# fenghuayumo/DIVSHOT

Measured on AMD Instinct MI355X. Metric: train views/sec (fwd+bwd raster) at 1M splats 1920x1080, higher is better.
Workload: dtype f32; 1 GPU; C3: 1000000 splats, 1920x1080, SH degree 3, 8 views per iteration sharded over 1 GPU(s) (BASELINE config C4), 8 view(s) per GPU per step as 1 multi-view pass(es) of 8 view(s) (dvs_raster_forward_views / dvs_raster_backward_*); absgrad=True, mode=batch, stagger=False, groups=1, views_per_group=8, early_gather=False, a9_chunks=1, async_forward=True, hip_graph=False, fwd_variant=quadrant, grad_mode=0, tile_bounds=canonical, shN_layout=tiled[N/64][45][64]

## Files before the change

### divshot_amd/csrc/dvs_api.cpp

```cpp
#include <hip/hip_runtime.h>
#include <cstdio>
#include <cstdlib>
#include <cstdint>
#include <cstring>
#include <mutex>
#include <string>
#include <vector>
#include "../../include/dvs_raster.h"
#include "dvs_kernels.h"

static thread_local std::string g_last_error;
static void set_error(const char* what, hipError_t e, const char* file, int line) {
    char buf[512];
    snprintf(buf, sizeof buf, "%s: %s (%s:%d)", what, hipGetErrorString(e), file, line);
    g_last_error = buf;
}
void dvs_set_last_error(const char* msg) { g_last_error = msg ? msg : ""; }
#define HIPCHECK(expr)                                                   \
    do {                                                                 \
        hipError_t _e = (expr);                                          \
        if (_e != hipSuccess) { set_error(#expr, _e, __FILE__, __LINE__); return DVS_ERR_HIP; } \
    } while (0)

namespace {
// ... 15 lines not shown
};

DvsCam to_dev_cam(const dvs_camera& c) {
    DvsCam d;
    memcpy(d.view, c.view, sizeof d.view); memcpy(d.proj, c.proj, sizeof d.proj);
    d.tan_fovx = c.tan_fovx; d.tan_fovy = c.tan_fovy; d.focal_x = c.focal_x; d.focal_y = c.focal_y;
    memcpy(d.campos, c.campos, sizeof d.campos);
    d.width = c.width; d.height = c.height; memcpy(d.bg, c.bg, sizeof d.bg);
    return d;
}
int bits_for(uint32_t max_value) { int b = 0; while (max_value) { ++b; max_value >>= 1; } return b; }
}

struct dvs_ctx {
    int device = 0;
    size_t max_splats = 0;
    int max_w = 0, max_h = 0;
    int max_views = 1;
    int n_views = 1;
    Buf radii, splat2d, depth, flags, tiles_touched, rect, rect_sorted, key[2], ids[2];
    Buf inst_tile[2], inst_splat[2];
    uint32_t* live_splat = nullptr;
    uint32_t* live_pos = nullptr;
    bool live_lists = true;
    Buf tmp_keys, tmp_vals;
    bool export_tiles = false;
    int fe_rank_atomic = 0;
    Buf ranges_canon;
    Buf ranges, final_T, n_contrib;
    size_t fe_zero_bytes = 0;
    uint32_t fe_nbv = 0, fe_nsb = 0;
    Buf fe_state;
    Buf fe_hist;
    int fe_seg_n = -1, fe_seg_V = -1;
    uint32_t fe_seg_rows = 0;
    Buf g_rows;
    Buf dcolor;
    uint64_t* total_dev = nullptr;
    uint64_t* total_host = nullptr;
    uint64_t inst_cap = 0;
    uint64_t inst_grow_events = 0;
    bool async_T = false;
    uint64_t* rec_masks = nullptr; uint64_t rec_cap = 0;
    uint64_t overflow_seen = 0;
    dvs_fwd_state st{};
    bool have_fwd = false;
    bool keep_rows = false;
    bool rows_clean = false;
    bool rows_pending = false;
    int64_t proj_next = 0;
    struct Prep {
// ... 67 lines not shown
    const size_t state = 3 * DVS_MAX_VIEWS * sizeof(DvsSeg) + ((size_t)c->max_views * c->fe_nsb + (size_t)c->max_views * DVS_FE_MAXBINS + (size_t)c->max_views * c->fe_nbv) * 4;
    if ((r = c->fe_state.ensure(state)) != DVS_OK) return r;
    if ((r = c->fe_hist.ensure(dvs_fe_hist_words((uint64_t)c->max_splats * c->max_views, c->max_views, DVS_FE_MAXBINS) * 4)) != DVS_OK) return r;
    return DVS_OK;
}

int ensure_splat_arenas(dvs_ctx* c, size_t n) {
    int r;
#define ENS(buf, bytes) if ((r = c->buf.ensure(bytes)) != DVS_OK) return r;
    ENS(radii, n * 4) ENS(splat2d, n * 64) ENS(depth, n * 4)
    ENS(flags, n * 4) ENS(tiles_touched, n * 4) ENS(rect, n * 16) ENS(rect_sorted, n * 16)      ENS(key[0], n * 4) ENS(key[1], n * 4) ENS(ids[0], n * 4) ENS(ids[1], n * 4)
    ENS(g_rows, n * 48)
#undef ENS
    return DVS_OK;
}
int ensure_image_arenas(dvs_ctx* c, int w, int h, int views) {
    const size_t P = (size_t)w * h * views;
    const size_t tiles = (size_t)((w + DVS_TILE - 1) / DVS_TILE) * ((h + DVS_TILE - 1) / DVS_TILE) * views;
    int r;
    if ((r = c->ranges.ensure(c->fe_zero_bytes + tiles * 8)) != DVS_OK) return r;
    if ((r = c->ranges_canon.ensure(tiles * 8)) != DVS_OK) return r;
    if ((r = c->final_T.ensure(P * 4)) != DVS_OK) return r;
    if ((r = c->n_contrib.ensure(P * 4)) != DVS_OK) return r;
    return DVS_OK;
}
int ensure_instance_arenas(dvs_ctx* c, uint64_t T) {
    int r;
    if (c->inst_cap && T > c->inst_cap) ++c->inst_grow_events;
    for (int k = 0; k < 2; ++k) {
        if ((r = c->inst_tile[k].ensure(T * 4)) != DVS_OK) return r;
        if ((r = c->inst_splat[k].ensure(T * 4)) != DVS_OK) return r;
    }
    c->inst_cap = c->inst_tile[0].bytes / 4;
    for (int k = 0; k < 2; ++k) {
        if (c->inst_tile[k].bytes / 4 < c->inst_cap) c->inst_cap = c->inst_tile[k].bytes / 4;
        if (c->inst_splat[k].bytes / 4 < c->inst_cap) c->inst_cap = c->inst_splat[k].bytes / 4;
    }
    if (c->inst_cap >= (1ull << 32)) c->inst_cap = (1ull << 32) - 1;
    if ((r = c->fe_hist.ensure(dvs_fe_hist_words(c->inst_cap, c->max_views, 512) * 4)) != DVS_OK) return r;
    return DVS_OK;
}
}

extern "C" {

const char* dvs_last_error(void) { return g_last_error.c_str(); }
// ... 33 lines not shown
                    hipMemcpy(&bad, word, 4, hipMemcpyDeviceToHost) == hipSuccess)
                    probed[device] = bad == 0u ? 1 : 2;
                if (word) (void)hipFree(word);
            }
            c->fe_rank_atomic = (device < 64 && probed[device] == 1) ? 1 : 0;
        }
    }
    if (const char* v = getenv("DVS_ASYNC")) c->async_T = v[0] == '1';
    if (ensure_frontend_arenas(c) != DVS_OK ||
        ensure_splat_arenas(c, max_splats * (size_t)max_views) != DVS_OK || ensure_image_arenas(c, max_w, max_h, max_views) != DVS_OK ||
        ensure_instance_arenas(c, (uint64_t)max_splats * 4 * (uint64_t)max_views) != DVS_OK) {
        dvs_destroy(c);
        return nullptr;
    }
    return c;
}
dvs_ctx* dvs_create(int device, size_t max_splats, int max_w, int max_h) { return dvs_create_views(device, max_splats, max_w, max_h, 1); }

void dvs_destroy(dvs_ctx* c) {
    if (!c) return;
    (void)hipSetDevice(c->device);
    Buf* all[] = {&c->radii, &c->splat2d, &c->depth, &c->flags, &c->tiles_touched, &c->rect, &c->rect_sorted, &c->key[0], &c->key[1],
                  &c->ids[0], &c->ids[1], &c->inst_tile[0], &c->inst_tile[1], &c->inst_splat[0], &c->inst_splat[1],
                  &c->tmp_keys, &c->tmp_vals, &c->ranges, &c->final_T, &c->n_contrib, &c->g_rows, &c->dcolor, &c->fe_state, &c->fe_hist, &c->ranges_canon};
    for (Buf* b : all) b->release();
    if (c->total_dev) (void)hipFree(c->total_dev);
    if (c->total_host) (void)hipHostFree(c->total_host);
    for (hipEvent_t e : c->events) (void)hipEventDestroy(e);
    for (hipEvent_t e : c->probe_ev) (void)hipEventDestroy(e);
    delete c;
}

static int rect_format(const dvs_opts* opts, int tiles_x, int tiles_y) {
    if (opts->tile_bounds == DVS_TILES_TIGHT) return DVS_FE_RECT_TIGHT;
    return (tiles_x <= 255 && tiles_y <= 255) ? DVS_FE_RECT_U8 : DVS_FE_RECT_U16;
}

static int run_a2(dvs_ctx* c, hipStream_t st, const dvs_splats* p, const dvs_camera* cams, int V, const dvs_opts* opts, int64_t first, int64_t count, bool begin) {
    const int n = p->n, W = cams[0].width, H = cams[0].height;
    const int tiles_x = (W + DVS_TILE - 1) / DVS_TILE, tiles_y = (H + DVS_TILE - 1) / DVS_TILE, tiles = tiles_x * tiles_y;
    const int rect_fmt = rect_format(opts, tiles_x, tiles_y);
    DvsCams dcams;
    for (int v = 0; v < V; ++v) dcams.c[v] = to_dev_cam(cams[v]);
    if (begin) HIPCHECK(hipMemsetAsync(c->ranges.p, 0, c->fe_zero_bytes + (size_t)tiles * V * 8, st));
    HIPCHECK(dvs_launch_preprocess_fwd(st, n, p->pos, p->sh0, p->shN, p->opacity, p->scale, p->rot, dcams, V, opts->sh_degree,
                                       opts->antialias, tiles_x, tiles_y, c->radii.as<int>(), c->splat2d.as<float>(),
                                       c->depth.as<float>(), c->flags.as<uint32_t>(), c->tiles_touched.as<uint32_t>(), c->key[0].as<uint32_t>(),
// ... 84 lines not shown
        if (n > 0)
            HIPCHECK(dvs_launch_seg_binning(st, n, V, rect_fmt, fe_seg_vis(c), fe_seg_tile(c), c->ids[1].as<uint32_t>(), c->rect.as<uint32_t>(),
                                            c->rect_sorted.as<uint32_t>(), fe_block_sums(c), fe_super(c), fe_superexcl(c), tile_part,
                                            (unsigned long long*)c->total_dev, c->inst_cap, 1, tiles_x, c->inst_tile[0].as<uint32_t>(),
                                            c->inst_splat[0].as<uint32_t>(), key16));
        size_t e5 = tm.mark(); tm.span("duplicate", e4, e5);
        const bool fuse_a6 = !fe_no_fuse();
        const bool write_keys = !(fuse_a6 && c->async_T) || c->export_tiles;
        if (n > 0) {
            const uint64_t cap = c->async_T ? c->inst_cap : T;
            const uint32_t nbtot = (uint32_t)(cap / tile_part) + (uint32_t)V + 2u;
            HIPCHECK(dvs_launch_seg_sort(st, V, c->inst_tile[0].as<uint32_t>(), c->inst_splat[0].as<uint32_t>(), c->inst_tile[1].as<uint32_t>(),
                                         c->inst_splat[1].as<uint32_t>(), fe_seg_tile(c), 0, tiles > 1 ? bits_for((uint32_t)(tiles - 1)) : 1,
                                         c->async_T ? (T_expected ? T_expected : c->inst_cap) : T, tile_part, nbtot, c->fe_hist.as<uint32_t>(), fe_totals(c),
                                         (uint32_t)tiles, &icur, fuse_a6 ? ranges_ptr(c) : nullptr, write_keys ? 1 : 0, key16, c->fe_rank_atomic));
        }
        size_t e6 = tm.mark(); tm.span("tile_sort", e5, e6);
        if (fuse_a6) ranges_encoded = n > 0 ? 1 : 0;
        else HIPCHECK(dvs_launch_tile_ranges(st, T, c->inst_tile[icur].as<uint32_t>(), ranges_ptr(c), T_dev, T_expected));
        keys_written = write_keys;
        e7 = tm.mark(); tm.span("tile_ranges", e6, e7);
    }
    if (c->probe) { (void)probe_event(c, st); c->probe_kind.push_back(0); }
    c->live_splat = nullptr; c->live_pos = nullptr;
    uint64_t* rec_masks = nullptr; uint64_t rec_cap = 0;
    if (c->rec_masks && V == 1 && !c->async_T) {
        rec_masks = c->rec_masks; rec_cap = c->rec_cap;
        HIPCHECK(hipMemsetAsync(rec_masks, 0, (size_t)(T < rec_cap ? T : rec_cap) * 32, st));
    }
    if (c->live_lists && c->bwd_variant == DVS_BWD_TR) { c->live_splat = c->inst_splat[icur ^ 1].as<uint32_t>(); c->live_pos = c->inst_tile[icur ^ 1].as<uint32_t>(); }
    HIPCHECK(dvs_launch_render_fwd(st, W, H, tiles_x, tiles_y, V, ranges_ptr(c), c->inst_splat[icur].as<uint32_t>(),
                                   c->splat2d.as<float>(), bgs, out_rgb, c->final_T.as<float>(), c->n_contrib.as<uint32_t>(),
                                   c->live_splat, c->live_pos, rec_masks, rec_cap, ranges_encoded ? c->ranges_canon.as<uint32_t>() : nullptr));
    if (c->probe) (void)probe_event(c, st);
    size_t e8 = tm.mark(); tm.span("render_fwd", e7, e8);

    dvs_fwd_state& s = c->st;
    s.radii = c->radii.as<int32_t>(); s.splat2d = c->splat2d.as<float>(); s.depth = c->depth.as<float>();
    s.flags = c->flags.as<uint32_t>();
    s.tiles_touched = c->tiles_touched.as<uint32_t>();
    s.sorted_tile = keys_written ? c->inst_tile[icur].as<uint32_t>() : nullptr; s.sorted_splat = c->inst_splat[icur].as<uint32_t>();
    s.ranges = ranges_encoded ? c->ranges_canon.as<uint32_t>() : ranges_ptr(c); s.final_T = c->final_T.as<float>(); s.n_contrib = c->n_contrib.as<uint32_t>();
    s.num_rendered = c->async_T ? DVS_T_UNKNOWN : T; s.n = n; s.width = W; s.height = H; s.tiles_x = tiles_x; s.tiles_y = tiles_y;
    s._pad = 0;
    c->n_views = V;
    c->have_fwd = true;
    if (saved) *saved = s;
    if (num_rendered) *num_rendered = c->async_T ? DVS_T_UNKNOWN : T;
    if (c->timing) { HIPCHECK(hipStreamSynchronize(st)); timing_collect(c, false); }
    return DVS_OK;
}

static int check_fwd_args(dvs_ctx* c, const dvs_splats* p, const dvs_camera* cams, int V, const dvs_opts* opts, const float* out_rgb) {
    if (!c || !p || !cams || !opts || !out_rgb) { g_last_error = "dvs_raster_forward: null argument"; return DVS_ERR_INVALID; }
    if (V < 1 || V > c->max_views) { g_last_error = "dvs_raster_forward: n_views exceeds the max_views given to dvs_create_views"; return DVS_ERR_CAPACITY; }
    const dvs_camera* cam = &cams[0];
// ... 66 lines not shown
    if (!c || !out) { g_last_error = "dvs_get_view_state: null argument"; return DVS_ERR_INVALID; }
    if (!c->have_fwd || view < 0 || view >= c->n_views) { g_last_error = "dvs_get_view_state: no such view in the last forward"; return DVS_ERR_STATE; }
    dvs_fwd_state s = c->st;
    const size_t on = (size_t)view * s.n, op = (size_t)view * s.width * s.height, ot = (size_t)view * s.tiles_x * s.tiles_y;
    s.radii += on; s.splat2d += on * DVS_S2D_FLOATS; s.depth += on; s.flags += on; s.tiles_touched += on;
    s.ranges += 2 * ot; s.final_T += op; s.n_contrib += op;
    *out = s;
    return DVS_OK;
}

static int bwd_composite(dvs_ctx* c, hipStream_t st, const dvs_camera* cams, const dvs_opts* opts, const float* dL_drgb, StageTimer* tm) {
    const dvs_fwd_state& s = c->st;
    const int V = c->n_views;
    size_t e0 = tm ? tm->mark() : 0;
    if (!c->rows_clean) HIPCHECK(hipMemsetAsync(c->g_rows.p, 0, c->g_rows.bytes, st));
    c->rows_clean = false;
    size_t e1 = tm ? tm->mark() : 0;
    if (tm) tm->span("bwd_zero", e0, e1);
    float bgs[DVS_MAX_VIEWS * 3];
    for (int v = 0; v < V; ++v) for (int k = 0; k < 3; ++k) bgs[3 * v + k] = cams[v].bg[k];
    if (c->probe) { (void)probe_event(c, st); c->probe_kind.push_back(1); }
    if (c->bwd_variant == DVS_BWD_TR)
        HIPCHECK(dvs_launch_render_bwd_tr(st, s.width, s.height, s.tiles_x, s.tiles_y, V, s.ranges, s.sorted_splat, s.splat2d, bgs, s.final_T,
                                          s.n_contrib, dL_drgb, c->g_rows.as<float>(), opts->absgrad, opts->grad_mode, c->live_splat, c->live_pos));
    else
        HIPCHECK(dvs_launch_render_bwd_blocks(st, s.width, s.height, s.tiles_x, s.tiles_y, V, s.ranges, s.sorted_splat, s.splat2d,
                                              bgs, s.final_T, s.n_contrib, dL_drgb, c->g_rows.as<float>(), opts->absgrad, opts->grad_mode));
    if (c->probe) (void)probe_event(c, st);
    if (tm) { size_t e2 = tm->mark(); tm->span("render_bwd", e1, e2); }
    c->rows_pending = true;
    c->proj_next = 0;
    return DVS_OK;
}
static int bwd_project(dvs_ctx* c, hipStream_t st, const dvs_splats* p, const dvs_camera* cams, const dvs_opts* opts,
                       const dvs_splat_grads* out, StageTimer* tm) {
    const dvs_fwd_state& s = c->st;
    const int V = c->n_views, n = p->n;
    size_t e2 = tm ? tm->mark() : 0;
    if (opts->shn_layout == DVS_SHN_TILED) {
        DvsCams dcams;
        float campos[DVS_MAX_VIEWS * 3];
        for (int v = 0; v < V; ++v) { dcams.c[v] = to_dev_cam(cams[v]); for (int k = 0; k < 3; ++k) campos[3 * v + k] = cams[v].campos[k]; }
        const char* nf = getenv("DVS_A9_NO_FUSE_SH");
        const bool no_fuse = nf && nf[0] == '1';
        const bool fuse = !out->dcolor && out->sh0 && out->shN && !no_fuse;
        float* dcol = out->dcolor;
        if (!dcol && !fuse) { int r = c->dcolor.ensure((size_t)V * n * 3 * sizeof(float)); if (r != DVS_OK) return r; dcol = c->dcolor.as<float>(); }
// ... 340 lines not shown

int dvs_memcpy_d2h(dvs_ctx* c, void* host_dst, const void* dev_src, size_t bytes) {
    if (!c) return DVS_ERR_INVALID;
    HIPCHECK(hipSetDevice(c->device));
    HIPCHECK(hipDeviceSynchronize());
    HIPCHECK(hipMemcpy(host_dst, dev_src, bytes, hipMemcpyDeviceToHost));
    return DVS_OK;
}
int dvs_memcpy_h2d(dvs_ctx* c, void* dev_dst, const void* host_src, size_t bytes) {
    if (!c) return DVS_ERR_INVALID;
    HIPCHECK(hipSetDevice(c->device));
    HIPCHECK(hipMemcpy(dev_dst, host_src, bytes, hipMemcpyHostToDevice));
    return DVS_OK;
}
void* dvs_device_malloc(dvs_ctx* c, size_t bytes) {
    if (!c) return nullptr;
    void* p = nullptr;
    if (hipSetDevice(c->device) != hipSuccess || hipMalloc(&p, bytes ? bytes : 1) != hipSuccess) return nullptr;
    return p;
}
void dvs_device_free(dvs_ctx* c, void* p) { if (c && p) { (void)hipSetDevice(c->device); (void)hipFree(p); } }

}
```

### divshot_amd/csrc/dvs_kernels.h

```cpp
#pragma once
#include <hip/hip_runtime.h>
#include <stdint.h>
#include "dvs_device.h"

hipError_t dvs_launch_preprocess_fwd(hipStream_t st, int n, const float* pos, const float* sh0, const float* shN,
                                     const float* opacity, const float* scale, const float* rot, const DvsCams& cams, int n_views,
                                     int deg, int antialias, int tiles_x, int tiles_y, int* radii , float* splat2d,
                                     float* depth, uint32_t* flags,
                                     uint32_t* tiles_touched, uint32_t* depth_key, int shn_tiled,
                                     uint32_t* rect , int rect_fmt ,
                                     uint32_t* kred ,
                                     int first, int count );
hipError_t dvs_launch_preprocess_bwd(hipStream_t st, int n, const float* pos, const float* shN, const float* opacity,
                                     const float* scale, const float* rot, const DvsCam& cam, int deg, int antialias,
                                     const int* radii, const uint32_t* flags, float* grad_rows ,
                                     float* g_pos, float* g_sh0, float* g_shN, float* g_opacity, float* g_scale,
                                     float* g_rot, float* out_absgrad2d , float* out_mean2d ,
                                     float* out_dcolor , int accumulate, int rezero_rows, int shn_tiled, int grad_mode);
hipError_t dvs_launch_preprocess_bwd_views(hipStream_t st, int n, int n_views, const float* pos, const float* shN, const float* opacity,
                                           const float* scale, const float* rot, const DvsCams& cams, int deg, int antialias,
                                           const int* radii, const uint32_t* flags, float* grad_rows, float* g_pos, float* g_opacity,
                                           float* g_scale, float* g_rot, float* out_absgrad2d, float* out_mean2d, float* out_dcolor,
                                           int accumulate, int rezero_rows, int grad_mode, int first = 0, int count = -1 ,
                                           float* g_sh0 = nullptr, float* g_shN = nullptr );
// ... 59 lines not shown
void dvs_fe_block_counts(int n, uint32_t* nbv, uint32_t* nsb);
hipError_t dvs_launch_seg_init(hipStream_t st, int n, int V, uint32_t rows_per_view, DvsSeg* seg_all);
hipError_t dvs_launch_depth_sort(hipStream_t st, int n, int V, uint32_t* keys0, uint32_t* vals0, uint32_t* keys1, uint32_t* vals1,
                                 DvsSeg* seg_all, DvsSeg* seg_vis, const uint32_t* kred, uint32_t* hist, uint32_t* totals ,
                                 int rank_atomic = 0 );
hipError_t dvs_launch_seg_sort(hipStream_t st, int V, uint32_t* keys0, uint32_t* vals0, uint32_t* keys1, uint32_t* vals1, DvsSeg* seg, int bit_lo, int bits,
                               uint64_t grid_elems, uint32_t part, uint32_t nbtot, uint32_t* hist, uint32_t* totals, uint32_t key_add_per_view,
                               int* result_in, uint32_t* ranges_enc = nullptr ,
                               int write_last_keys = 1, int first_keys16 = 0 , int rank_atomic = 0);
hipError_t dvs_fe_probe_rank_atomic(hipStream_t st, uint32_t* bad_dev);
hipError_t dvs_launch_seg_binning(hipStream_t st, int n, int V, int rect_fmt, const DvsSeg* seg_vis, DvsSeg* seg_tile, const uint32_t* sorted_ids,
                                  const uint32_t* rect, uint32_t* rect_sorted, uint32_t* block_sums, unsigned long long* super, uint32_t* superexcl,
                                  uint32_t tile_part, unsigned long long* total_dev, unsigned long long capacity, int stage, int tiles_x,
                                  uint32_t* inst_tile, uint32_t* inst_splat, int key16 = 0 );

hipError_t dvs_launch_tile_ranges(hipStream_t st, uint64_t T, const uint32_t* sorted_tile, uint32_t* ranges ,
                                  const uint64_t* T_dev = nullptr, uint64_t T_expected = 0);
hipError_t dvs_launch_export_keys(hipStream_t st, uint64_t T, const uint32_t* sorted_tile, const uint32_t* sorted_splat,
                                  const float* depth, uint64_t* out_keys);

hipError_t dvs_launch_render_fwd(hipStream_t st, int W, int H, int tiles_x, int tiles_y, int n_views, const uint32_t* ranges ,
                                 const uint32_t* sorted_splat, const float* splat2d, const float* bgs, float* out_color, float* final_T,
                                 uint32_t* n_contrib, uint32_t* live_splat , uint32_t* live_pos ,
                                 uint64_t* take_masks ,
                                 uint64_t take_cap, uint32_t* ranges_out = nullptr );
enum { DVS_BWD_BLOCKS = 0 , DVS_BWD_REDUCE = 1 , DVS_BWD_MM = 2 ,
       DVS_BWD_TR = 3  };

hipError_t dvs_launch_render_bwd_tr(hipStream_t st, int W, int H, int tiles_x, int tiles_y, int n_views, const uint32_t* ranges,
                                    const uint32_t* sorted_splat, const float* splat2d, const float* bgs , const float* final_T,
                                    const uint32_t* n_contrib, const float* dL_dout, float* grad_rows, int absgrad, int grad_mode,
                                    const uint32_t* live_splat ,
                                    const uint32_t* live_pos);

hipError_t dvs_launch_render_bwd_blocks(hipStream_t st, int W, int H, int tiles_x, int tiles_y, int n_views, const uint32_t* ranges,
                                        const uint32_t* sorted_splat, const float* splat2d, const float* bgs , const float* final_T,
                                        const uint32_t* n_contrib, const float* dL_dout, float* grad_rows, int absgrad, int grad_mode);
```

### divshot_amd/csrc/render.hip

```cpp
#include "dvs_device.h"
#include "dvs_kernels.h"
#include "render_common.h"

struct __attribute__((aligned(16))) FwdLds {
    float4 a[RB];
    float4 b[RB];
    float4 c[RB];
    uint64_t qmask[RB / 64][4];
    uint32_t wlive[RB / 64];
};
__device__ __forceinline__ void lds_put(FwdLds& L, int t, float2 xy, float4 co, float3 col) {
    L.a[t] = make_float4(xy.x, xy.y, -0.72134752044448170f * co.x, -1.4426950408889634f * co.y);
    L.b[t] = make_float4(-0.72134752044448170f * co.z, co.w, col.x, col.y);
    L.c[t].x = col.z;
}

__device__ __forceinline__ bool stage_batch(FwdLds& L, const uint32_t* __restrict__ sorted_splat, uint32_t first, int cnt,
                                            const float4* __restrict__ splat2d, float tile_x0, float tile_y0, uint32_t& id_out) {
    const int t = threadIdx.x;
    uint32_t qm = 0;
    id_out = 0u;
    if (t < cnt) {
        const uint32_t id = sorted_splat[first + t];
        id_out = id;
// ... 29 lines not shown
        }
    }
    const uint64_t m0 = __ballot(qm & 1u), m1 = __ballot(qm & 2u), m2 = __ballot(qm & 4u), m3 = __ballot(qm & 8u);
    if ((t & 63) == 0) {
        uint64_t* dst = L.qmask[t >> 6];
        dst[0] = m0; dst[1] = m1; dst[2] = m2; dst[3] = m3;
    }
    return qm != 0u;
}

__device__ __forceinline__ uint64_t uniform_u64(uint64_t v) {
    const uint32_t lo = __builtin_amdgcn_readfirstlane((uint32_t)v), hi = __builtin_amdgcn_readfirstlane((uint32_t)(v >> 32));
    return ((uint64_t)hi << 32) | lo;
}

template <bool RECORD>
__global__ void __launch_bounds__(RB)
k_render_fwd(ViewBg bg_arg , int W, int H, int tiles_x, int tiles_per_view,
             int num_tiles , const uint2* __restrict__ ranges, uint2* __restrict__ ranges_out ,
             const uint32_t* __restrict__ sorted_splat, const float4* __restrict__ splat2d,
             float* __restrict__ out_color , float* __restrict__ final_T , uint32_t* __restrict__ n_contrib,
             uint32_t* __restrict__ live_splat ,
             uint32_t* __restrict__ live_pos ,
             uint64_t* __restrict__ take_masks , uint64_t take_cap) {
    __shared__ FwdLds L;
    (void)bg_arg;
    const int tile_g = tile_of_block(blockIdx.x, num_tiles);
    if (tile_g >= num_tiles) return;
    const int view = tile_g / tiles_per_view, tile = tile_g - view * tiles_per_view;
    const float3 bgv = dvs_load_bg(view);
    const float bg0 = bgv.x, bg1 = bgv.y, bg2 = bgv.z;
    out_color += (size_t)view * 3 * W * H; final_T += (size_t)view * W * H; n_contrib += (size_t)view * W * H;
    const int tx = tile % tiles_x, ty = tile / tiles_x;
    const int wave = threadIdx.x >> 6, lane = threadIdx.x & 63;
    const int px = tx * DVS_TILE + (wave & 1) * 8 + (lane & 7);
    const int py = ty * DVS_TILE + (wave >> 1) * 8 + (lane >> 3);
    const bool inside = px < W && py < H;
    const float pxf = (float)px, pyf = (float)py;
    uint2 range = ranges[tile_g];
    if (ranges_out) {
        range.x = range.y ? ~range.x : 0u;
        if (threadIdx.x == 0) ranges_out[tile_g] = range;
    }
    const int total = (int)(range.y - range.x);
    uint64_t notdone = __builtin_amdgcn_ballot_w64(inside);
    float T = 1.0f, C0 = 0.f, C1 = 0.f, C2 = 0.f;
// ... 51 lines not shown
                             "v_cmpx_ngt_f32_e32 vcc, %[amin], %[al]\n\t"
                             "v_cmp_gt_f32_e32 vcc, %[tstop], %[tt]\n\t"
                             "s_andn2_b64 %[nd], %[nd], vcc\n\t"
                             "s_andn2_b64 exec, exec, vcc\n\t"
                             "v_fmac_f32 %[c0], %[cr], %[at]\n\t"
                             "v_fmac_f32 %[c1], %[cg], %[at]\n\t"
                             "v_fmac_f32 %[c2], %[cbl], %[at]\n\t"
                             "v_sub_f32 %[T], %[T], %[at]\n\t"
                             "v_mov_b32 %[last], %[idx]\n\t"
                             "s_mov_b64 exec, %[ee]"
                             : [c0] "+v"(C0), [c1] "+v"(C1), [c2] "+v"(C2), [T] "+v"(T), [last] "+v"(last), [nd] "+s"(notdone)
                             : [p2] "v"(p2), [al] "v"(alpha), [tt] "v"(test_T), [cr] "v"(B.z), [cg] "v"(B.w), [cbl] "v"(cb), [at] "v"(aT), [idx] "s"(idx),
                               [amin] "s"(DVS_ALPHA_MIN), [tstop] "s"(DVS_T_STOP), [ee] "s"(exec_entry)
                             : "vcc", "scc");
                if (RECORD) {
                    const uint64_t took = nd_before & __builtin_amdgcn_ballot_w64(!(p2 > 0.f)) & __builtin_amdgcn_ballot_w64(!(alpha < DVS_ALPHA_MIN)) &
                                          ~__builtin_amdgcn_ballot_w64(test_T < DVS_T_STOP);
                    const uint64_t pos = (uint64_t)range.x + (uint64_t)(idx - 1u);
                    if (lane == 0 && pos < take_cap) take_masks[pos * 4 + wave] = took;
                }
            }
        }
    }
    if (inside) {
        const size_t P = (size_t)W * H, pix = (size_t)py * W + px;
        final_T[pix] = T;
        n_contrib[pix] = last;
        out_color[pix] = C0 + T * bg0;
        out_color[P + pix] = C1 + T * bg1;
        out_color[2 * P + pix] = C2 + T * bg2;
    }
}


hipError_t dvs_launch_render_fwd(hipStream_t st, int W, int H, int tiles_x, int tiles_y, int n_views, const uint32_t* ranges,
                                 const uint32_t* sorted_splat, const float* splat2d, const float* bgs, float* out_color, float* final_T,
                                 uint32_t* n_contrib, uint32_t* live_splat, uint32_t* live_pos, uint64_t* take_masks, uint64_t take_cap, uint32_t* ranges_out) {
    const int tiles_pv = tiles_x * tiles_y, num_tiles = tiles_pv * n_views;
    if (num_tiles <= 0) return hipSuccess;
    const int grid = ((num_tiles + 7) >> 3) << 3;
    if (take_masks)
        hipLaunchKernelGGL(k_render_fwd<true>, dim3(grid), dim3(RB), 0, st, make_view_bg(n_views, bgs), W, H, tiles_x, tiles_pv, num_tiles,
                           (const uint2*)ranges, (uint2*)ranges_out, sorted_splat, (const float4*)splat2d, out_color, final_T, n_contrib, live_splat, live_pos, take_masks, take_cap);
    else
        hipLaunchKernelGGL(k_render_fwd<false>, dim3(grid), dim3(RB), 0, st, make_view_bg(n_views, bgs), W, H, tiles_x, tiles_pv, num_tiles,
                           (const uint2*)ranges, (uint2*)ranges_out, sorted_splat, (const float4*)splat2d, out_color, final_T, n_contrib, live_splat, live_pos, (uint64_t*)nullptr, (uint64_t)0);
    return hipGetLastError();
}
```

### divshot_amd/csrc/render_tr.hip

```cpp
#include "dvs_device.h"
#include "dvs_kernels.h"
#include "render_common.h"

#define TR_SLOTS 4
#define TR_SS 136
#define TR_MINW 6

template <int BK>
struct __attribute__((aligned(16))) TrLds {
    float4 ea[BK + 1];
    float4 eb[BK + 1];
    float4 ec[BK + 1];
    uint2 idop[2][BK];
    uint8_t list[(BK + 1) * 16];
    uint32_t cnt[16];
    uint32_t blast[16];
};

template <int BK>
__device__ __forceinline__ uint32_t tr_load_id(const uint32_t* __restrict__ sorted_splat, uint32_t first, int cnt) {
    const int e = threadIdx.x % BK;
    return e < cnt ? sorted_splat[first + e] : 0u;
}
template <int BK>
// ... 40 lines not shown
        uint32_t rk, len;
        if (BK == 64) {
            rk = __builtin_amdgcn_mbcnt_hi((uint32_t)(m >> 32), __builtin_amdgcn_mbcnt_lo((uint32_t)m, 0u));
            len = (uint32_t)__popcll(m);
        } else {
            const uint32_t lo = (uint32_t)m, hi = (uint32_t)(m >> 32);
            const bool up = lane >= 32;
            rk = up ? __builtin_amdgcn_mbcnt_hi(hi, 0u) : __builtin_amdgcn_mbcnt_lo(lo, 0u);
            len = (uint32_t)__popc(up ? hi : lo);
        }
        if (hit) L.list[(rk + 1u) * 16u + (uint32_t)(b0 + i)] = (uint8_t)e;
        if (e == 0) L.cnt[b0 + i] = len;
    }
}

template <bool ABSGRAD, bool LINEAGE, int BK>
__global__ void __launch_bounds__(RB, TR_MINW)
k_render_bwd_tr(ViewBg bg_arg , int W, int H, int tiles_x, int tiles_per_view,
                int num_tiles , const uint2* __restrict__ ranges,
                const uint32_t* __restrict__ sorted_splat, const float4* __restrict__ splat2d,
                const float* __restrict__ final_T, const uint32_t* __restrict__ n_contrib, const float* __restrict__ dL_dout ,
                float* __restrict__ grow ,
                const uint32_t* __restrict__ live_splat ,
                const uint32_t* __restrict__ live_pos ) {
    __shared__ TrLds<BK> L;
    __shared__ __attribute__((aligned(16))) float s_tab[4][(BK + 1) * 12];
    __shared__ __attribute__((aligned(16))) float s_tb[4][TR_SLOTS * TR_SS];
    (void)bg_arg;
    const int tile_g = tile_of_block(blockIdx.x, num_tiles);
    if (tile_g >= num_tiles) return;
    const int view = tile_g / tiles_per_view, tile = tile_g - view * tiles_per_view;
    const float3 bgv = dvs_load_bg(view);
    final_T += (size_t)view * W * H; n_contrib += (size_t)view * W * H; dL_dout += (size_t)view * 3 * W * H;
    const int tx = tile % tiles_x, ty = tile / tiles_x;
    const int wave = threadIdx.x >> 6, lane = threadIdx.x & 63;
    const size_t P = (size_t)W * H;
    const int g1 = lane >> 4, pi = lane & 15;
    const int bx1 = 2 * (wave & 1) + (g1 & 1), by1 = 2 * (wave >> 1) + (g1 >> 1), blk1 = by1 * 4 + bx1;
    const int px = tx * DVS_TILE + 4 * bx1 + (pi & 3), py = ty * DVS_TILE + 4 * by1 + (pi >> 2);
    const bool inside = px < W && py < H;
    const size_t pix = (size_t)py * W + px;
    const float pxf = (float)px, pyf = (float)py;
    const uint2 range = ranges[tile_g];
    const int r2 = lane >> 4, s2 = (lane >> 2) & 3, g2 = lane & 3;
    const int bx2 = 2 * (wave & 1) + (g2 & 1), by2 = 2 * (wave >> 1) + (g2 >> 1);
    const int X0 = tx * DVS_TILE + 4 * bx2, Y0 = ty * DVS_TILE + 4 * by2 + r2;
    const float X0f = (float)X0, Y0f = (float)Y0;
    float d2[4][3];
    if ((W & 3) == 0) {
        const bool in2 = X0 < W && Y0 < H;
        const size_t q = (size_t)Y0 * W + X0;
#pragma unroll
        for (int c = 0; c < 3; ++c) {
            const float4 v = in2 ? *reinterpret_cast<const float4*>(dL_dout + c * P + q) : make_float4(0.f, 0.f, 0.f, 0.f);
            d2[0][c] = v.x; d2[1][c] = v.y; d2[2][c] = v.z; d2[3][c] = v.w;
        }
    } else {
#pragma unroll
        for (int x = 0; x < 4; ++x) {
            const bool in2 = X0 + x < W && Y0 < H;
            const size_t q = (size_t)Y0 * W + X0 + x;
#pragma unroll
            for (int c = 0; c < 3; ++c) d2[x][c] = in2 ? dL_dout[c * P + q] : 0.f;
        }
    }
    const int perm_r = (r2 == 1) ? 2 : (r2 == 2) ? 1 : r2;
    const int xaddr = (lane ^ 32) << 2;
    const int jaddr = (16 * g2) << 2;
    const uint32_t jshift = 8u * (uint32_t)(TR_SLOTS - 1 - s2);

    const float T_final = inside ? final_T[pix] : 0.f;
    uint32_t last = inside ? n_contrib[pix] : 0u;
    if (live_pos) {
        if (last > 0u) last = live_pos[range.x + last - 1u] + 1u;
        sorted_splat = live_splat;
    }
    float dLp0 = 0.f, dLp1 = 0.f, dLp2 = 0.f;
    if (inside) { dLp0 = dL_dout[pix]; dLp1 = dL_dout[P + pix]; dLp2 = dL_dout[2 * P + pix]; }
    const float bg_dot = (bgv.x * dLp0 + bgv.y * dLp1) + bgv.z * dLp2;

    uint32_t bmax = last;
#pragma unroll
    for (int d = 8; d >= 1; d >>= 1) bmax = max(bmax, (uint32_t)__shfl_xor((int)bmax, d, 64));
    if (pi == 0) L.blast[blk1] = bmax;
    for (int e = threadIdx.x; e < (BK + 1) * 12; e += RB) reinterpret_cast<float4*>(&s_tab[0][0])[e] = make_float4(0.f, 0.f, 0.f, 0.f);
    if (threadIdx.x < 16) L.list[threadIdx.x] = (uint8_t)BK;
    if (threadIdx.x == 0) { L.ea[BK] = make_float4(0.f, 0.f, 0.f, 0.f); L.eb[BK] = make_float4(0.f, 0.f, 0.f, 0.f); L.ec[BK] = make_float4(0.f, 0.f, 0.f, 0.f); }
    __syncthreads();
    uint32_t todo = 0;
#pragma unroll
    for (int g = 0; g < 16; ++g) todo = max(todo, L.blast[g]);
    if (todo == 0) return;

    float T = T_final;
    float D = T_final * bg_dot;
    const uint32_t tb_m0 = (uint32_t)__builtin_amdgcn_readfirstlane((int)(uint32_t)(uintptr_t)&s_tb[wave][0]);
    typedef __attribute__((address_space(3))) float lds_float;
    typedef float tr_v4f __attribute__((ext_vector_type(4)));
    typedef __attribute__((address_space(3))) const tr_v4f lds_cv4f;
    uint32_t tbr_a = (uint32_t)(uintptr_t)&s_tb[wave][TR_SS * s2 + 16 * g2 + 4 * r2];
    uint32_t tabw_a = (uint32_t)(uintptr_t)&s_tab[wave][perm_r];
    asm("" : "+v"(tbr_a), "+v"(tabw_a));
    const uint8_t* const lbase = &L.list[0];

    auto flush = [&](uint32_t jpack) {
        const uint32_t jp = (uint32_t)__builtin_amdgcn_ds_bpermute(jaddr, (int)jpack);
        const int j = (int)((jp >> jshift) & 0xffu);
        const tr_v4f V_ = *(lds_cv4f*)tbr_a, W_ = *(lds_cv4f*)(tbr_a + 256u);
        const float4 V = make_float4(V_.x, V_.y, V_.z, V_.w), Wv = make_float4(W_.x, W_.y, W_.z, W_.w);
        const float2 mean = *reinterpret_cast<const float2*>(&L.ea[j]);
        const float4 cq = L.ec[j];
        asm("" : : "v"(cq.x));
        const float Dx = mean.x - X0f, Dy = mean.y - Y0f;
        const float A0 = (V.x + V.y) + (V.z + V.w);
        const float B0 = __builtin_fmaf(3.f, V.w, __builtin_fmaf(2.f, V.z, V.y));
// ... 20 lines not shown
        const float h3 = swap32_add(v[6], v[7]);
        float h4, h5;
        if (ABSGRAD) {
            h4 = swap32_add(v[8], v[9]);
            h5 = v[10] + __int_as_float(__builtin_amdgcn_ds_bpermute(xaddr, __float_as_int(v[10])));
        } else {
            h4 = v[8] + __int_as_float(__builtin_amdgcn_ds_bpermute(xaddr, __float_as_int(v[8])));
            h5 = 0.f;
        }
        const float q0 = swap16_add(h0, h1), q1 = swap16_add(h2, h3), q2 = swap16_add(h4, h5);
        uint32_t slot_a;
        asm("v_mad_u32_u24 %0, %1, 48, %2" : "=v"(slot_a) : "v"(j), "v"(tabw_a));
        lds_float* const slot = (lds_float*)slot_a;
#pragma unroll
        for (int g = 0; g < 4; ++g) {
            if (g2 == g) { slot[0] += q0; slot[4] += q1; slot[8] += q2; }
            __builtin_amdgcn_wave_barrier();
            asm volatile("" ::: "memory");
        }
    };

    const int nbatch = (int)((todo + BK - 1) / BK);
    const float tile_x0 = (float)(tx * DVS_TILE), tile_y0 = (float)(ty * DVS_TILE);
    uint32_t id_stage = tr_load_id<BK>(sorted_splat, range.x + (nbatch - 1) * BK, min(BK, (int)todo - (nbatch - 1) * BK));
    for (int b = nbatch - 1; b >= 0; --b) {
        const int base = b * BK;
        const int cnt = min(BK, (int)todo - base);
        tr_stage<BK>(L, splat2d, id_stage, cnt, base, b & 1, tile_x0, tile_y0);
        __syncthreads();
        const int len = (int)L.cnt[blk1];
        int nmax = len;
        nmax = max(nmax, __shfl_xor(nmax, 16, 64));
        nmax = max(nmax, __shfl_xor(nmax, 32, 64));
        nmax = __builtin_amdgcn_readfirstlane(nmax);
        const int lastb = (int)min(last, (uint32_t)(base + BK)) - base;
        uint32_t p = (uint32_t)len * 16u + (uint32_t)blk1;
        uint32_t jn = lbase[p];
        asm("" : "+v"(jn));
        uint32_t jpack = 0;
        int nslot = 0;
#pragma unroll 1
        for (int it = 0; it < nmax; ++it) {
            const int j = (int)jn;
            jpack = (jpack << 8) | (uint32_t)j;
            const bool below_last = j < lastb;
            const float4 ea = L.ea[j];
            const float4 eb = L.eb[j];
// ... 27 lines not shown
                tbw[TR_SS * nslot] = 0.f; tbw[TR_SS * nslot + 64] = 0.f;
                jpack = (jpack << 8) | (uint32_t)BK;
            }
            flush(jpack);
        }
        __syncthreads();
        if (b > 0) id_stage = tr_load_id<BK>(sorted_splat, range.x + (b - 1) * BK, BK);
        for (int e = threadIdx.x; e < cnt * 12; e += RB) {
            const float val = (s_tab[0][e] + s_tab[1][e]) + (s_tab[2][e] + s_tab[3][e]);
            if (val != 0.f) {
                const int ent = e / 12, comp = e - 12 * ent;
                const uint2 io = L.idop[b & 1][ent];
                const float sc = (comp == 5 || (comp >= 6 && comp <= 8)) ? 1.f : __uint_as_float(io.y);
                if (comp < 11) atomicAdd(&grow[(size_t)io.x * 12 + comp], val * sc);
            }
            s_tab[0][e] = 0.f; s_tab[1][e] = 0.f; s_tab[2][e] = 0.f; s_tab[3][e] = 0.f;
        }
    }
}

hipError_t dvs_launch_render_bwd_tr(hipStream_t st, int W, int H, int tiles_x, int tiles_y, int n_views, const uint32_t* ranges,
                                    const uint32_t* sorted_splat, const float* splat2d, const float* bgs, const float* final_T,
                                    const uint32_t* n_contrib, const float* dL_dout, float* grad_rows, int absgrad, int grad_mode,
                                    const uint32_t* live_splat, const uint32_t* live_pos) {
    const int tiles_pv = tiles_x * tiles_y, num_tiles = tiles_pv * n_views;
    if (num_tiles <= 0) return hipSuccess;
    const int grid = ((num_tiles + 7) >> 3) << 3;
    const int lineage = grad_mode == 1 ? 1 : 0;
#define DVS_TR(A, LN, BKV)                                                                                                              \
    hipLaunchKernelGGL((k_render_bwd_tr<A, LN, BKV>), dim3(grid), dim3(RB), 0, st, make_view_bg(n_views, bgs), W, H, tiles_x, tiles_pv, \
                       num_tiles, (const uint2*)ranges, sorted_splat, (const float4*)splat2d, final_T, n_contrib, dL_dout, grad_rows, live_splat, live_pos)
#define DVS_TR_B(BKV)                                                                                   \
    do {                                                                                                \
        if (absgrad) { if (lineage) DVS_TR(true, true, BKV); else DVS_TR(true, false, BKV); }           \
        else { if (lineage) DVS_TR(false, true, BKV); else DVS_TR(false, false, BKV); }                 \
    } while (0)
    DVS_TR_B(64);
#undef DVS_TR_B
#undef DVS_TR
    return hipGetLastError();
}
```

Before: 1824 views/s.

## Hand off live-list pixel counts and per-block maxima from forward to backward

The forward render now converts each pixel's contributor count into a live-list position and writes it to a new per-pixel buffer. It also reduces per-4x4-block maxima and writes them to a per-tile array. The backward tile kernel reads these precomputed values instead of doing a dependent gather through live_pos, a shuffle reduction and an LDS pass. This lets it exit early for empty tiles and prefetch the first id batch before the barrier. The cost is extra global writes and a barrier in the forward pass, plus two new image-sized buffers.

```diff
diff --git a/divshot_amd/csrc/dvs_api.cpp b/divshot_amd/csrc/dvs_api.cpp
--- a/divshot_amd/csrc/dvs_api.cpp
+++ b/divshot_amd/csrc/dvs_api.cpp
@@ -61,11 +61,14 @@
     Buf inst_tile[2], inst_splat[2];
     uint32_t* live_splat = nullptr;
     uint32_t* live_pos = nullptr;
+    uint32_t* n_contrib_live = nullptr;
+    uint32_t* tile_blast = nullptr;
     bool live_lists = true;
     Buf tmp_keys, tmp_vals;
     bool export_tiles = false;
     int fe_rank_atomic = 0;
     Buf ranges_canon;
+    Buf handoff_px, handoff_tile;
     Buf ranges, final_T, n_contrib;
     size_t fe_zero_bytes = 0;
     uint32_t fe_nbv = 0, fe_nsb = 0;
@@ -179,6 +182,8 @@
     if ((r = c->ranges_canon.ensure(tiles * 8)) != DVS_OK) return r;
     if ((r = c->final_T.ensure(P * 4)) != DVS_OK) return r;
     if ((r = c->n_contrib.ensure(P * 4)) != DVS_OK) return r;
+    if ((r = c->handoff_px.ensure(P * 4)) != DVS_OK) return r;
+    if ((r = c->handoff_tile.ensure(tiles * 64)) != DVS_OK) return r;
     return DVS_OK;
 }
 int ensure_instance_arenas(dvs_ctx* c, uint64_t T) {
@@ -258,7 +263,8 @@
     (void)hipSetDevice(c->device);
     Buf* all[] = {&c->radii, &c->splat2d, &c->depth, &c->flags, &c->tiles_touched, &c->rect, &c->rect_sorted, &c->key[0], &c->key[1],
                   &c->ids[0], &c->ids[1], &c->inst_tile[0], &c->inst_tile[1], &c->inst_splat[0], &c->inst_splat[1],
-                  &c->tmp_keys, &c->tmp_vals, &c->ranges, &c->final_T, &c->n_contrib, &c->g_rows, &c->dcolor, &c->fe_state, &c->fe_hist, &c->ranges_canon};
+                  &c->tmp_keys, &c->tmp_vals, &c->ranges, &c->final_T, &c->n_contrib, &c->g_rows, &c->dcolor, &c->fe_state, &c->fe_hist, &c->ranges_canon,
+                  &c->handoff_px, &c->handoff_tile};
     for (Buf* b : all) b->release();
     if (c->total_dev) (void)hipFree(c->total_dev);
     if (c->total_host) (void)hipHostFree(c->total_host);
@@ -389,16 +395,19 @@
         e7 = tm.mark(); tm.span("tile_ranges", e6, e7);
     }
     if (c->probe) { (void)probe_event(c, st); c->probe_kind.push_back(0); }
-    c->live_splat = nullptr; c->live_pos = nullptr;
+    c->live_splat = nullptr; c->live_pos = nullptr; c->n_contrib_live = nullptr; c->tile_blast = nullptr;
     uint64_t* rec_masks = nullptr; uint64_t rec_cap = 0;
     if (c->rec_masks && V == 1 && !c->async_T) {
         rec_masks = c->rec_masks; rec_cap = c->rec_cap;
         HIPCHECK(hipMemsetAsync(rec_masks, 0, (size_t)(T < rec_cap ? T : rec_cap) * 32, st));
     }
-    if (c->live_lists && c->bwd_variant == DVS_BWD_TR) { c->live_splat = c->inst_splat[icur ^ 1].as<uint32_t>(); c->live_pos = c->inst_tile[icur ^ 1].as<uint32_t>(); }
+    if (c->live_lists && c->bwd_variant == DVS_BWD_TR) {
+        c->live_splat = c->inst_splat[icur ^ 1].as<uint32_t>(); c->live_pos = c->inst_tile[icur ^ 1].as<uint32_t>();
+        c->n_contrib_live = c->handoff_px.as<uint32_t>(); c->tile_blast = c->handoff_tile.as<uint32_t>();
+    }
     HIPCHECK(dvs_launch_render_fwd(st, W, H, tiles_x, tiles_y, V, ranges_ptr(c), c->inst_splat[icur].as<uint32_t>(),
                                    c->splat2d.as<float>(), bgs, out_rgb, c->final_T.as<float>(), c->n_contrib.as<uint32_t>(),
-                                   c->live_splat, c->live_pos, rec_masks, rec_cap, ranges_encoded ? c->ranges_canon.as<uint32_t>() : nullptr));
+                                   c->live_splat, c->live_pos, c->n_contrib_live, c->tile_blast, rec_masks, rec_cap, ranges_encoded ? c->ranges_canon.as<uint32_t>() : nullptr));
     if (c->probe) (void)probe_event(c, st);
     size_t e8 = tm.mark(); tm.span("render_fwd", e7, e8);
 
@@ -511,7 +520,8 @@
     if (c->probe) { (void)probe_event(c, st); c->probe_kind.push_back(1); }
     if (c->bwd_variant == DVS_BWD_TR)
         HIPCHECK(dvs_launch_render_bwd_tr(st, s.width, s.height, s.tiles_x, s.tiles_y, V, s.ranges, s.sorted_splat, s.splat2d, bgs, s.final_T,
-                                          s.n_contrib, dL_drgb, c->g_rows.as<float>(), opts->absgrad, opts->grad_mode, c->live_splat, c->live_pos));
+                                          s.n_contrib, dL_drgb, c->g_rows.as<float>(), opts->absgrad, opts->grad_mode, c->live_splat, c->live_pos,
+                                          c->n_contrib_live, c->tile_blast));
     else
         HIPCHECK(dvs_launch_render_bwd_blocks(st, s.width, s.height, s.tiles_x, s.tiles_y, V, s.ranges, s.sorted_splat, s.splat2d,
                                               bgs, s.final_T, s.n_contrib, dL_drgb, c->g_rows.as<float>(), opts->absgrad, opts->grad_mode));
@@ -898,3 +908,13 @@
 void dvs_device_free(dvs_ctx* c, void* p) { if (c && p) { (void)hipSetDevice(c->device); (void)hipFree(p); } }
 
 }
+
+namespace dvs_test {
+__attribute__((visibility("default"))) int handoff_state(dvs_ctx* c, const uint32_t** live_pos, const uint32_t** n_contrib_live, const uint32_t** tile_blast) {
+    if (!c || !c->have_fwd) return DVS_ERR_STATE;
+    if (live_pos) *live_pos = c->live_pos;
+    if (n_contrib_live) *n_contrib_live = c->n_contrib_live;
+    if (tile_blast) *tile_blast = c->tile_blast;
+    return DVS_OK;
+}
+}
diff --git a/divshot_amd/csrc/dvs_kernels.h b/divshot_amd/csrc/dvs_kernels.h
--- a/divshot_amd/csrc/dvs_kernels.h
+++ b/divshot_amd/csrc/dvs_kernels.h
@@ -105,6 +105,7 @@
 hipError_t dvs_launch_render_fwd(hipStream_t st, int W, int H, int tiles_x, int tiles_y, int n_views, const uint32_t* ranges ,
                                  const uint32_t* sorted_splat, const float* splat2d, const float* bgs, float* out_color, float* final_T,
                                  uint32_t* n_contrib, uint32_t* live_splat , uint32_t* live_pos ,
+                                 uint32_t* n_contrib_live , uint32_t* tile_blast ,
                                  uint64_t* take_masks ,
                                  uint64_t take_cap, uint32_t* ranges_out = nullptr );
 enum { DVS_BWD_BLOCKS = 0 , DVS_BWD_REDUCE = 1 , DVS_BWD_MM = 2 ,
@@ -114,7 +115,7 @@
                                     const uint32_t* sorted_splat, const float* splat2d, const float* bgs , const float* final_T,
                                     const uint32_t* n_contrib, const float* dL_dout, float* grad_rows, int absgrad, int grad_mode,
                                     const uint32_t* live_splat ,
-                                    const uint32_t* live_pos);
+                                    const uint32_t* live_pos, const uint32_t* n_contrib_live , const uint32_t* tile_blast);
 
 hipError_t dvs_launch_render_bwd_blocks(hipStream_t st, int W, int H, int tiles_x, int tiles_y, int n_views, const uint32_t* ranges,
                                         const uint32_t* sorted_splat, const float* splat2d, const float* bgs , const float* final_T,
diff --git a/divshot_amd/csrc/render.hip b/divshot_amd/csrc/render.hip
--- a/divshot_amd/csrc/render.hip
+++ b/divshot_amd/csrc/render.hip
@@ -75,6 +75,8 @@
              float* __restrict__ out_color , float* __restrict__ final_T , uint32_t* __restrict__ n_contrib,
              uint32_t* __restrict__ live_splat ,
              uint32_t* __restrict__ live_pos ,
+             uint32_t* __restrict__ n_contrib_live ,
+             uint32_t* __restrict__ tile_blast ,
              uint64_t* __restrict__ take_masks , uint64_t take_cap) {
     __shared__ FwdLds L;
     (void)bg_arg;
@@ -172,8 +174,23 @@
             }
         }
     }
+    const size_t P = (size_t)W * H, pix = (size_t)py * W + px;
+    if (n_contrib_live) {
+        __threadfence_block();
+        __syncthreads();
+        const uint32_t ll = last ? live_pos[range.x + last - 1u] + 1u : 0u;
+        if (inside) n_contrib_live[(size_t)view * P + pix] = ll;
+        uint32_t bmax = ll;
+        bmax = max(bmax, (uint32_t)__shfl_xor((int)bmax, 1, 64));
+        bmax = max(bmax, (uint32_t)__shfl_xor((int)bmax, 2, 64));
+        bmax = max(bmax, (uint32_t)__shfl_xor((int)bmax, 8, 64));
+        bmax = max(bmax, (uint32_t)__shfl_xor((int)bmax, 16, 64));
+        if ((lane & 27) == 0) {
+            const int bx = 2 * (wave & 1) + ((lane >> 2) & 1), by = 2 * (wave >> 1) + (lane >> 5);
+            tile_blast[(size_t)tile_g * 16 + (size_t)(by * 4 + bx)] = bmax;
+        }
+    }
     if (inside) {
-        const size_t P = (size_t)W * H, pix = (size_t)py * W + px;
         final_T[pix] = T;
         n_contrib[pix] = last;
         out_color[pix] = C0 + T * bg0;
@@ -185,15 +202,17 @@
 
 hipError_t dvs_launch_render_fwd(hipStream_t st, int W, int H, int tiles_x, int tiles_y, int n_views, const uint32_t* ranges,
                                  const uint32_t* sorted_splat, const float* splat2d, const float* bgs, float* out_color, float* final_T,
-                                 uint32_t* n_contrib, uint32_t* live_splat, uint32_t* live_pos, uint64_t* take_masks, uint64_t take_cap, uint32_t* ranges_out) {
+                                 uint32_t* n_contrib, uint32_t* live_splat, uint32_t* live_pos, uint32_t* n_contrib_live, uint32_t* tile_blast,
+                                 uint64_t* take_masks, uint64_t take_cap, uint32_t* ranges_out) {
     const int tiles_pv = tiles_x * tiles_y, num_tiles = tiles_pv * n_views;
     if (num_tiles <= 0) return hipSuccess;
     const int grid = ((num_tiles + 7) >> 3) << 3;
+    if (!live_pos || !n_contrib_live || !tile_blast) { n_contrib_live = nullptr; tile_blast = nullptr; }
     if (take_masks)
         hipLaunchKernelGGL(k_render_fwd<true>, dim3(grid), dim3(RB), 0, st, make_view_bg(n_views, bgs), W, H, tiles_x, tiles_pv, num_tiles,
-                           (const uint2*)ranges, (uint2*)ranges_out, sorted_splat, (const float4*)splat2d, out_color, final_T, n_contrib, live_splat, live_pos, take_masks, take_cap);
+                           (const uint2*)ranges, (uint2*)ranges_out, sorted_splat, (const float4*)splat2d, out_color, final_T, n_contrib, live_splat, live_pos, n_contrib_live, tile_blast, take_masks, take_cap);
     else
         hipLaunchKernelGGL(k_render_fwd<false>, dim3(grid), dim3(RB), 0, st, make_view_bg(n_views, bgs), W, H, tiles_x, tiles_pv, num_tiles,
-                           (const uint2*)ranges, (uint2*)ranges_out, sorted_splat, (const float4*)splat2d, out_color, final_T, n_contrib, live_splat, live_pos, (uint64_t*)nullptr, (uint64_t)0);
+                           (const uint2*)ranges, (uint2*)ranges_out, sorted_splat, (const float4*)splat2d, out_color, final_T, n_contrib, live_splat, live_pos, n_contrib_live, tile_blast, (uint64_t*)nullptr, (uint64_t)0);
     return hipGetLastError();
 }
diff --git a/divshot_amd/csrc/render_tr.hip b/divshot_amd/csrc/render_tr.hip
--- a/divshot_amd/csrc/render_tr.hip
+++ b/divshot_amd/csrc/render_tr.hip
@@ -86,7 +86,9 @@
                 const float* __restrict__ final_T, const uint32_t* __restrict__ n_contrib, const float* __restrict__ dL_dout ,
                 float* __restrict__ grow ,
                 const uint32_t* __restrict__ live_splat ,
-                const uint32_t* __restrict__ live_pos ) {
+                const uint32_t* __restrict__ live_pos ,
+                const uint32_t* __restrict__ n_contrib_live ,
+                const uint32_t* __restrict__ tile_blast ) {
     __shared__ TrLds<BK> L;
     __shared__ __attribute__((aligned(16))) float s_tab[4][(BK + 1) * 12];
     __shared__ __attribute__((aligned(16))) float s_tb[4][TR_SLOTS * TR_SS];
@@ -106,6 +108,14 @@
     const size_t pix = (size_t)py * W + px;
     const float pxf = (float)px, pyf = (float)py;
     const uint2 range = ranges[tile_g];
+    const bool handoff = tile_blast != nullptr;
+    uint32_t todo = 0, id_stage = 0, blast_t = 0;
+    if (handoff) {
+        const uint32_t* const bl = tile_blast + (size_t)tile_g * 16;
+#pragma unroll
+        for (int g = 0; g < 16; ++g) todo = max(todo, bl[g]);
+        if (todo == 0) return;
+    }
     const int r2 = lane >> 4, s2 = (lane >> 2) & 3, g2 = lane & 3;
     const int bx2 = 2 * (wave & 1) + (g2 & 1), by2 = 2 * (wave >> 1) + (g2 >> 1);
     const int X0 = tx * DVS_TILE + 4 * bx2, Y0 = ty * DVS_TILE + 4 * by2 + r2;
@@ -128,33 +138,45 @@
             for (int c = 0; c < 3; ++c) d2[x][c] = in2 ? dL_dout[c * P + q] : 0.f;
         }
     }
+    if (handoff) {
+        sorted_splat = live_splat;
+        id_stage = tr_load_id<BK>(sorted_splat, range.x + ((todo - 1u) / BK) * BK, (int)((todo - 1u) % BK) + 1);
+        if (threadIdx.x < 16) blast_t = tile_blast[(size_t)tile_g * 16 + threadIdx.x];
+    }
     const int perm_r = (r2 == 1) ? 2 : (r2 == 2) ? 1 : r2;
     const int xaddr = (lane ^ 32) << 2;
     const int jaddr = (16 * g2) << 2;
     const uint32_t jshift = 8u * (uint32_t)(TR_SLOTS - 1 - s2);
 
     const float T_final = inside ? final_T[pix] : 0.f;
-    uint32_t last = inside ? n_contrib[pix] : 0u;
-    if (live_pos) {
-        if (last > 0u) last = live_pos[range.x + last - 1u] + 1u;
-        sorted_splat = live_splat;
+    uint32_t last;
+    if (handoff) last = inside ? (n_contrib_live + (size_t)view * W * H)[pix] : 0u;
+    else {
+        last = inside ? n_contrib[pix] : 0u;
+        if (live_pos) {
+            if (last > 0u) last = live_pos[range.x + last - 1u] + 1u;
+            sorted_splat = live_splat;
+        }
     }
     float dLp0 = 0.f, dLp1 = 0.f, dLp2 = 0.f;
     if (inside) { dLp0 = dL_dout[pix]; dLp1 = dL_dout[P + pix]; dLp2 = dL_dout[2 * P + pix]; }
     const float bg_dot = (bgv.x * dLp0 + bgv.y * dLp1) + bgv.z * dLp2;
 
-    uint32_t bmax = last;
-#pragma unroll
-    for (int d = 8; d >= 1; d >>= 1) bmax = max(bmax, (uint32_t)__shfl_xor((int)bmax, d, 64));
-    if (pi == 0) L.blast[blk1] = bmax;
+    if (!handoff) {
+        uint32_t bmax = last;
+#pragma unroll
+        for (int d = 8; d >= 1; d >>= 1) bmax = max(bmax, (uint32_t)__shfl_xor((int)bmax, d, 64));
+        if (pi == 0) L.blast[blk1] = bmax;
+    } else if (threadIdx.x < 16) L.blast[threadIdx.x] = blast_t;
     for (int e = threadIdx.x; e < (BK + 1) * 12; e += RB) reinterpret_cast<float4*>(&s_tab[0][0])[e] = make_float4(0.f, 0.f, 0.f, 0.f);
     if (threadIdx.x < 16) L.list[threadIdx.x] = (uint8_t)BK;
     if (threadIdx.x == 0) { L.ea[BK] = make_float4(0.f, 0.f, 0.f, 0.f); L.eb[BK] = make_float4(0.f, 0.f, 0.f, 0.f); L.ec[BK] = make_float4(0.f, 0.f, 0.f, 0.f); }
     __syncthreads();
-    uint32_t todo = 0;
-#pragma unroll
-    for (int g = 0; g < 16; ++g) todo = max(todo, L.blast[g]);
-    if (todo == 0) return;
+    if (!handoff) {
+#pragma unroll
+        for (int g = 0; g < 16; ++g) todo = max(todo, L.blast[g]);
+        if (todo == 0) return;
+    }
 
     float T = T_final;
     float D = T_final * bg_dot;
@@ -221,7 +243,7 @@
 
     const int nbatch = (int)((todo + BK - 1) / BK);
     const float tile_x0 = (float)(tx * DVS_TILE), tile_y0 = (float)(ty * DVS_TILE);
-    uint32_t id_stage = tr_load_id<BK>(sorted_splat, range.x + (nbatch - 1) * BK, min(BK, (int)todo - (nbatch - 1) * BK));
+    if (!handoff) id_stage = tr_load_id<BK>(sorted_splat, range.x + (nbatch - 1) * BK, min(BK, (int)todo - (nbatch - 1) * BK));
     for (int b = nbatch - 1; b >= 0; --b) {
         const int base = b * BK;
         const int cnt = min(BK, (int)todo - base);
@@ -295,14 +317,17 @@
 hipError_t dvs_launch_render_bwd_tr(hipStream_t st, int W, int H, int tiles_x, int tiles_y, int n_views, const uint32_t* ranges,
                                     const uint32_t* sorted_splat, const float* splat2d, const float* bgs, const float* final_T,
                                     const uint32_t* n_contrib, const float* dL_dout, float* grad_rows, int absgrad, int grad_mode,
-                                    const uint32_t* live_splat, const uint32_t* live_pos) {
+                                    const uint32_t* live_splat, const uint32_t* live_pos, const uint32_t* n_contrib_live,
+                                    const uint32_t* tile_blast) {
+    if (!live_splat || !live_pos || !n_contrib_live || !tile_blast) { n_contrib_live = nullptr; tile_blast = nullptr; }
     const int tiles_pv = tiles_x * tiles_y, num_tiles = tiles_pv * n_views;
     if (num_tiles <= 0) return hipSuccess;
     const int grid = ((num_tiles + 7) >> 3) << 3;
     const int lineage = grad_mode == 1 ? 1 : 0;
 #define DVS_TR(A, LN, BKV)                                                                                                              \
     hipLaunchKernelGGL((k_render_bwd_tr<A, LN, BKV>), dim3(grid), dim3(RB), 0, st, make_view_bg(n_views, bgs), W, H, tiles_x, tiles_pv, \
-                       num_tiles, (const uint2*)ranges, sorted_splat, (const float4*)splat2d, final_T, n_contrib, dL_dout, grad_rows, live_splat, live_pos)
+                       num_tiles, (const uint2*)ranges, sorted_splat, (const float4*)splat2d, final_T, n_contrib, dL_dout, grad_rows, live_splat, live_pos, \
+                       n_contrib_live, tile_blast)
 #define DVS_TR_B(BKV)                                                                                   \
     do {                                                                                                \
         if (absgrad) { if (lineage) DVS_TR(true, true, BKV); else DVS_TR(true, false, BKV); }           \
```

Result: no change. 1814 views/s (-0.6%).
